# MannLabs/alphadia

Hardware: AMD Instinct MI355X
Metric: precursors scored/sec (higher is better)
Workload: dtype f32/f64; 1 GPU; 1000000-precursor predicted library x 3 candidates vs 2h synthetic Thermo-style DIA run (4800 cycles x 61 spectra); BASELINE configs[2] on one GPU; precursors_total=1000000, candidates_total=3000000, candidates_per_gpu=3000000, cycles=4800, parallelism=single GPU, rccl_ranks_seen=1, priming_steps_before_warmup=4

## Files before the change

### alphadia_amd/csrc/adh_copyout.hip

```cpp

__global__ void adh_slot_count_kernel(const uint16_t *__restrict__ lib_slot, int64_t row0, int64_t n, int top_k,
                                      uint32_t *__restrict__ cnt) {
    const int64_t i = (int64_t)blockIdx.x * blockDim.x + threadIdx.x;
    if (i > n) return;
    uint32_t k = 0;
    if (i < n) {
        const uint16_t *s = lib_slot + (row0 + i) * (int64_t)top_k;
        while (k < (uint32_t)top_k && s[k]) ++k;
    }
    cnt[i] = k;
}

#include "adh_fill_host.h"

struct PadLayout {
    size_t per_row, total;
    PadLayout(int64_t n, int top_k, int64_t n_chunks)
        : per_row(4 + (size_t)top_k * 22), total(base(n, n_chunks + 1, 4 + (size_t)top_k * 22) + 64) {}
    size_t base(int64_t a, int64_t ci) const { return base(a, ci, per_row); }
    static size_t base(int64_t a, int64_t ci, size_t per_row_) {
        return ((size_t)a * per_row_ + ((size_t)(a / kAnchorRows) + (size_t)ci) * 8 + (size_t)ci * 1024 + 255) & ~(size_t)255;
    }
};

// ... 39 lines not shown
        const uint16_t *s = lib_slot + r0;
        for (; v.s < (uint32_t)top_k && s[v.s]; ++v.s) {
            v.i += intensity[r0 + v.s] != 0u;
            v.c += correlation[r0 + v.s] != 0u;
            v.big += s[v.s] >= big_from;
        }
    }
    cnt[i] = v;
}

__global__ void adh_pad_pack_sparse_kernel(DevOut t, int64_t row0, int64_t n, int top_k, const SlotCnt *__restrict__ scan,
                                           unsigned char *__restrict__ block, uint32_t *__restrict__ totals) {
    const int64_t id = (int64_t)blockIdx.x * blockDim.x + threadIdx.x;
    const SlotCnt tot = scan[n];
    const bool sparse = tot.big == 0;
    const SparseBlock L((uint64_t)row0, (uint64_t)n, tot.s, tot.i, tot.c, sparse);
    uint32_t *const off = reinterpret_cast<uint32_t *>(block + L.off);
    if (id == 0) {
        const uint32_t head[4] = {sparse ? kWireSparse : kWireDense, tot.s, tot.i, tot.c};
        for (int q = 0; q < 4; ++q) reinterpret_cast<uint32_t *>(block)[q] = head[q], totals[q] = head[q];
        off[n] = tot.s;
    }
    const bool in_table = id < n * top_k;
    const int64_t i = in_table ? id / top_k : 0;
    const int j = in_table ? (int)(id - i * top_k) : 0;
    SlotCnt a{0, 0, 0, 0};
    uint32_t k = 0;
    if (in_table) {
        a = scan[i];
        k = scan[i + 1].s - a.s;
        if (j == 0) {
            off[i] = a.s;
            if (sparse && (row0 + i) % kAnchorRows == 0) {
                uint32_t *anchor = reinterpret_cast<uint32_t *>(block + L.anchor) +
                                   2 * ((row0 + i) / kAnchorRows - (int64_t)SparseBlock::anchor_row0((uint64_t)row0));
                anchor[0] = a.i, anchor[1] = a.c;
            }
        }
    }
    const bool filled = in_table && (uint32_t)j < k;
    const int64_t src = (row0 + i) * (int64_t)top_k + j;
    const uint32_t *const intensity = reinterpret_cast<const uint32_t *>(t.fragment_intensity);
    const uint32_t *const correlation = reinterpret_cast<const uint32_t *>(t.fragment_correlation);
    const uint32_t vi = filled ? intensity[src] : 0u, vc = filled ? correlation[src] : 0u;
    const uint64_t nz_i = __ballot(vi != 0u), nz_c = __ballot(vc != 0u);
    if (!filled) return;
    const size_t dst = (size_t)a.s + (size_t)j;
    uint16_t word = t.fragment_lib_slot[src];
    size_t di = dst, dc = dst;
    if (sparse) {
        uint32_t pi = a.i, pc = a.c;
        const int lane = (int)(threadIdx.x & (ADH_WAVE - 1));
        if (j <= lane) {
            const uint64_t before = ((1ull << j) - 1ull) << (lane - j);
            pi += (uint32_t)__popcll(nz_i & before), pc += (uint32_t)__popcll(nz_c & before);
        } else {
            for (int q = 0; q < j; ++q) pi += intensity[src - j + q] != 0u, pc += correlation[src - j + q] != 0u;
        }
        di = pi, dc = pc;
        word |= (vi ? kHasIntensity : 0u) | (vc ? kHasCorrelation : 0u);
    }
    reinterpret_cast<uint16_t *>(block + L.slot)[dst] = word;
    reinterpret_cast<float *>(block + L.f[0])[dst] = t.fragment_mz_observed[src];
    reinterpret_cast<float *>(block + L.f[1])[dst] = t.fragment_height[src];
    reinterpret_cast<float *>(block + L.f[3])[dst] = t.fragment_mass_error[src];
    if (!sparse || vi) reinterpret_cast<uint32_t *>(block + L.f[2])[di] = vi;
    if (!sparse || vc) reinterpret_cast<uint32_t *>(block + L.f[4])[dc] = vc;
}

__global__ void adh_cop_count_kernel(const uint8_t *__restrict__ valid, const uint16_t *__restrict__ lib_slot, int64_t row0,
                                     int64_t n, int top_k, uint64_t *__restrict__ cnt) {
    const int64_t i = (int64_t)blockIdx.x * blockDim.x + threadIdx.x;
    if (i > n) return;
    uint64_t v = 0;
    if (i < n && valid[row0 + i]) {
        const uint16_t *s = lib_slot + (row0 + i) * (int64_t)top_k;
        uint32_t k = 0;
        while (k < (uint32_t)top_k && s[k]) ++k;
        v = (1ull << 32) | k;
    }
    cnt[i] = v;
}

struct CopBlock {
    size_t row, cnt, feat, s_slot, s_f[5], total;
    __host__ __device__ CopBlock(uint64_t R, uint64_t S) {
        size_t o = 0;
        row = o, o += (R * 4 + 15) & ~(size_t)15;
        cnt = o, o += (R + 15) & ~(size_t)15;
        feat = o, o += (R * 4 * ADH_NUM_FEATURES + 15) & ~(size_t)15;
        s_slot = o, o += (S * 2 + 15) & ~(size_t)15;
        for (int j = 0; j < 5; ++j) s_f[j] = o, o += (S * 4 + 15) & ~(size_t)15;
        total = o;
    }
};
struct CopLayout {
    size_t per_row, total;
    CopLayout(int64_t n, int top_k, int64_t n_chunks)
        : per_row(5 + 4 * ADH_NUM_FEATURES + (size_t)top_k * 22), total((size_t)n * per_row + (size_t)(n_chunks + 1) * 1024) {}
    size_t base(int64_t a, int64_t ci) const { return ((size_t)a * per_row + (size_t)ci * 1024 + 255) & ~(size_t)255; }
};

__global__ void adh_cop_pack_kernel(DevOut t, DevCands c, const LibRec *__restrict__ lib, int64_t row0, int64_t n, int top_k,
                                    const uint64_t *__restrict__ off, unsigned char *__restrict__ block,
                                    uint64_t *__restrict__ totals) {
    const int64_t stride = (int64_t)gridDim.x * blockDim.x;
    const int64_t tid = (int64_t)blockIdx.x * blockDim.x + threadIdx.x;
    const uint64_t tot = off[n];
    const uint64_t R = tot >> 32, S = tot & 0xFFFFFFFFull;
    if (tid == 0) totals[0] = tot;
    const CopBlock L(R, S);
    uint32_t *const o_row = reinterpret_cast<uint32_t *>(block + L.row);
    uint8_t *const o_cnt = block + L.cnt;
    float *const o_feat = reinterpret_cast<float *>(block + L.feat);
    for (int64_t i = tid; i < n; i += stride) {
        const uint64_t o = off[i], o1 = off[i + 1];
        if ((o1 >> 32) == (o >> 32)) continue;
        const int64_t j = (int64_t)(o >> 32), r = row0 + i;
        o_row[j] = (uint32_t)r;
        o_cnt[j] = (uint8_t)((uint32_t)o1 - (uint32_t)o);
        const float *f = t.features + r * ADH_NUM_FEATURES;
#pragma unroll
        for (int k = 0; k < ADH_NUM_FEATURES; ++k) o_feat[(size_t)k * R + (size_t)j] = f[k];
    }
    uint16_t *const s_slot = reinterpret_cast<uint16_t *>(block + L.s_slot);
    const int64_t n_slots = n * (int64_t)top_k;
    for (int64_t id = tid; id < n_slots; id += stride) {
        const int64_t i = id / top_k;
        const int s = (int)(id - i * top_k);
        const uint64_t o = off[i], o1 = off[i + 1];
        const uint32_t a = (uint32_t)o, k = (uint32_t)o1 - a;
        if ((uint32_t)s >= k) continue;
        const int64_t r = row0 + i, src = r * (int64_t)top_k + s;
        const size_t dst = (size_t)a + (size_t)s;
        s_slot[dst] = t.fragment_lib_slot[src];
        reinterpret_cast<float *>(block + L.s_f[0])[dst] = t.fragment_mz_observed[src];
        reinterpret_cast<float *>(block + L.s_f[1])[dst] = t.fragment_height[src];
        reinterpret_cast<float *>(block + L.s_f[2])[dst] = t.fragment_intensity[src];
        reinterpret_cast<float *>(block + L.s_f[3])[dst] = t.fragment_mass_error[src];
        reinterpret_cast<float *>(block + L.s_f[4])[dst] = t.fragment_correlation[src];
    }
}

namespace {
void cop_copy_stripe(const unsigned char *block, int64_t cnt_r, int64_t cnt_s, int64_t base_r, int64_t base_s,
                     adh_compact_output_t *out, int w, int T, const adh_candidates_t *c, const LibRec *lib) {
    const CopBlock L((uint64_t)cnt_r, (uint64_t)cnt_s);
    const int64_t lo = cnt_r * w / T, hi = cnt_r * (w + 1) / T;
    if (hi <= lo) return;
    const uint32_t *rows = reinterpret_cast<const uint32_t *>(block + L.row);
    const uint8_t *cnt = block + L.cnt;
    int64_t s_lo = 0;
    for (int64_t j = 0; j < lo; ++j) s_lo += cnt[j];
    memcpy(out->row + base_r + lo, rows + lo, (size_t)(hi - lo) * 4);
    const float *fb = reinterpret_cast<const float *>(block + L.feat);
    for (int k = 0; k < ADH_NUM_FEATURES; ++k)
        memcpy(out->features + (size_t)k * (size_t)out->rows_capacity + (size_t)(base_r + lo),
               fb + (size_t)k * (size_t)cnt_r + (size_t)lo, (size_t)(hi - lo) * 4);
    const uint16_t *slot = reinterpret_cast<const uint16_t *>(block + L.s_slot);
    int64_t d = base_s + s_lo, at = s_lo;
    for (int64_t j = lo; j < hi; ++j) {
        const uint32_t r = rows[j];
        const uint32_t p = c->precursor_idx[r];
        const uint8_t rk = c->rank ? c->rank[r] : (uint8_t)0;
        out->precursor_idx[base_r + j] = p;
        out->rank[base_r + j] = rk;
        const LibRec *base = lib + c->frag_start_idx[r];
        const int k = (int)cnt[j];
        for (int q = 0; q < k; ++q, ++d, ++at) {
            const LibRec &l = base[slot[at] - 1];
            out->fragment_row[d] = r;
            out->fragment_precursor_idx[d] = p;
            out->fragment_rank[d] = rk;
            out->fragment_mz_library[d] = l.mz_library;
            out->fragment_mz[d] = l.mz;
            out->fragment_position[d] = l.position;
            out->fragment_number[d] = l.number;
            out->fragment_type[d] = l.type;
            out->fragment_charge[d] = l.charge;
            out->fragment_loss_type[d] = l.loss_type;
        }
    }
    const size_t m = (size_t)(at - s_lo);
    if (m) {
        float *const fcol[5] = {out->fragment_mz_observed, out->fragment_height, out->fragment_intensity, out->fragment_mass_error,
                                out->fragment_correlation};
        for (int j = 0; j < 5; ++j) memcpy(fcol[j] + base_s + s_lo, block + L.s_f[j] + (size_t)s_lo * 4, m * 4);
    }
}

void rebuild_host_rows(const adh_handle *h, const adh_candidates_t *c, adh_output_t *out, const uint16_t *slots,
                       int64_t a, int64_t b) {
    const int top_k = out->top_k;
    const LibRec *lib = h->h_lib.data();
    for (int64_t i = a; i < b; ++i) {
        const bool skip = c->flags && (c->flags[i] & ADH_FLAG_SKIP);
        const uint32_t p = skip ? 0u : c->precursor_idx[i];
        const uint8_t r = skip ? (uint8_t)0 : c->rank[i];
        out->precursor_idx[i] = p;
        out->rank[i] = r;
        const LibRec *base = lib + c->frag_start_idx[i];
        for (int j = 0; j < top_k; ++j) {
            const size_t o = (size_t)i * (size_t)top_k + (size_t)j;
            const uint16_t s = slots[o];
            if (s) {
                const LibRec &l = base[s - 1];
                out->fragment_precursor_idx[o] = p;
                out->fragment_rank[o] = r;
                out->fragment_mz_library[o] = l.mz_library;
                out->fragment_mz[o] = l.mz;
                out->fragment_position[o] = l.position;
                out->fragment_number[o] = l.number;
                out->fragment_type[o] = l.type;
                out->fragment_charge[o] = l.charge;
                out->fragment_loss_type[o] = l.loss_type;
            } else {
                out->fragment_precursor_idx[o] = 0;
                out->fragment_rank[o] = 0;
                out->fragment_mz_library[o] = 0.0f;
                out->fragment_mz[o] = 0.0f;
                out->fragment_position[o] = 0;
                out->fragment_number[o] = 0;
                out->fragment_type[o] = 0;
                out->fragment_charge[o] = 0;
                out->fragment_loss_type[o] = 0;
            }
        }
    }
}

int host_thread_share() {
    int t = 16;
    if (const char *env = getenv("ADH_HOST_THREADS")) t = atoi(env);
    else {
        int ranks = 1;
        if (const char *lw = getenv("LOCAL_WORLD_SIZE")) ranks = std::max(atoi(lw), 1);
        t = std::min<int>(t, std::max<int>(host_cpu_budget() / ranks, 1));
    }
    return std::max(t, 1);
}

int host_threads_for(int64_t n) {
    const int t = (int)std::min<int64_t>(host_thread_share(), n / 16384);
    return std::max(t, 1);
}

bool host_rebuild_pays() {
    int least = 6;
    if (const char *env = getenv("ADH_REBUILD_MIN_THREADS")) least = atoi(env);
    return host_thread_share() >= least;
}

bool compact_copy_out_pays(int64_t n) {
    if (const char *env = getenv("ADH_COMPACT_COPY_OUT")) return atoi(env) != 0;
    int64_t least_rows = 1000000;
    if (const char *env = getenv("ADH_COMPACT_MIN_ROWS")) least_rows = atoll(env);
    return host_thread_share() >= 12 && n >= least_rows;
}

bool sparse_slots_pay(int64_t n) {
    if (const char *env = getenv("ADH_SPARSE_SLOTS")) return atoi(env) != 0;
    int64_t least_rows = 1000000;
    if (const char *env = getenv("ADH_SPARSE_SLOTS_MIN_ROWS")) least_rows = atoll(env);
    return n >= least_rows;
}

struct BlockHandoff {
    std::vector<hipEvent_t> events;
    std::atomic<int64_t> appended{0}, ready{0};
    std::atomic<bool> watching{false}, abort{false};
    hipError_t error = hipSuccess;
    int device = 0;
    std::function<void(int64_t)> landed;
// ... 375 lines not shown
        const int64_t a = cut[(size_t)ci], b = cut[(size_t)ci + 1];
        const double t_in = trace.stripe_begin();
        for (;;) {
            const int64_t t = a / kFillTile + next_tile[(size_t)ci].fetch_add(1, std::memory_order_relaxed);
            const int64_t lo = std::max(a, t * kFillTile), hi = std::min(b, (t + 1) * kFillTile);
            if (lo >= b) break;
            fill_host_rows(h->h_lib.data(), c, out, host_blocks + lay.base(a, ci), b - a, a, lo, hi, sparse);
        }
        trace.stripe_end(ci, w, t_in);
    }
    void start_team() override {
        (void)start_handoff_team(team, T, n_chunks, [this](int64_t ci, int w) { stripe(ci, w); });
    }
    int pack(int64_t ci) override {
        const int64_t a = cut[(size_t)ci], nr = cut[(size_t)ci + 1] - a;
        hipStream_t sk = h->stream;
        unsigned char *blk = dev_blocks + lay.base(a, ci);
        if (sparse) {
            SlotCnt *cnt = static_cast<SlotCnt *>(h->cmp_cnt);
            hipLaunchKernelGGL(adh_slot_count_nz_kernel, dim3((unsigned)((nr + 256) / 256)), dim3(256), 0, sk, dev.fragment_lib_slot,
                               reinterpret_cast<const uint32_t *>(dev.fragment_intensity),
                               reinterpret_cast<const uint32_t *>(dev.fragment_correlation), a, nr, top_k, big_from, cnt);
            size_t scan_bytes = h->cmp_scan_bytes;
            HIP_TRY(hipcub::DeviceScan::ExclusiveScan(h->cmp_scan, scan_bytes, cnt, cnt, SlotCntSum(), SlotCnt{0, 0, 0, 0},
                                                      (int)(nr + 1), sk));
            hipLaunchKernelGGL(adh_pad_pack_sparse_kernel, dim3((unsigned)((nr * top_k + 255) / 256)), dim3(256), 0, sk, dev, a, nr,
                               top_k, cnt, blk, h->cmp_tot_pinned + 4 * ci);
            HIP_TRY(hipGetLastError());
            return record(sk, tot_ready);
        }
        uint32_t *d_off = reinterpret_cast<uint32_t *>(blk);
        hipLaunchKernelGGL(adh_slot_count_kernel, dim3((unsigned)((nr + 256) / 256)), dim3(256), 0, sk, dev.fragment_lib_slot, a,
                           nr, top_k, d_off);
        size_t scan_bytes = h->cmp_scan_bytes;
        HIP_TRY(hipcub::DeviceScan::ExclusiveSum(h->cmp_scan, scan_bytes, d_off, d_off, (int)(nr + 1), sk));
        hipLaunchKernelGGL(adh_pad_pack_kernel, dim3((unsigned)((nr * top_k + 255) / 256)), dim3(256), 0, sk, dev, a, nr, top_k,
                           blk, h->cmp_tot_pinned + ci);
        HIP_TRY(hipGetLastError());
        return record(sk, tot_ready);
    }
    int send(int64_t ci) {
        const int64_t a = cut[(size_t)ci], b = cut[(size_t)ci + 1];
        HIP_TRY(hipEventSynchronize(tot_ready[(size_t)ci]));
        trace.total_seen(ci);
        const size_t base = lay.base(a, ci);
        size_t bytes = 0;
        if (sparse) {
            const uint32_t *tot = h->cmp_tot_pinned + 4 * ci;
            bytes = SparseBlock((uint64_t)a, (uint64_t)(b - a), tot[1], tot[2], tot[3], tot[0] == kWireSparse).total;
            wire_slots += tot[1], wire_nz_i += tot[0] == kWireSparse ? tot[2] : tot[1], wire_nz_c += tot[0] == kWireSparse ? tot[3] : tot[1];
        } else {
            bytes = PadBlock((uint64_t)(b - a), (uint64_t)h->cmp_tot_pinned[ci]).total;
        }
        h->d2h_bytes += bytes;
        trace.block_sent(ci, bytes, PadBlock((uint64_t)(b - a), sparse ? h->cmp_tot_pinned[4 * ci + 1] : h->cmp_tot_pinned[ci]).total);
        return send_block(handoff, host_blocks + base, dev_blocks + base, bytes);
    }
    int copy_out(int64_t ci) override {
        if (ci == 0) {
            HIP_TRY(hipStreamWaitEvent(h->stream_out, h->ev_k[0], 0));
            return copy_tables(0, false);
        }
        int rc = send(ci - 1);
        if (rc == ADH_OK && ci > 1) rc = copy_tables(ci - 1, false);
        return rc;
    }
    int flush() override { return copy_out(n_chunks); }
    int finish() override {
        if (!handoff.wait_for(n_chunks - 1))
            return fail(ADH_ERR_HIP, std::string("scoring pipeline (compacted copy-out): ") + hipGetErrorString(handoff.error));
        for (int64_t ci = 0; ci < n_chunks; ++ci) stripe(ci, T);
        team.join_all();
        if (trace.timing)
            fprintf(stderr, "[adh]   compacted copy-out: host team done %.2f ms after the call began (%d threads)\n", trace.since(), T);
        if (trace.timing && sparse)
            fprintf(stderr, "[adh]   sparse-slot wire: %llu filled slots, %llu intensity words and %llu correlation words sent\n",
                    (unsigned long long)wire_slots, (unsigned long long)wire_nz_i, (unsigned long long)wire_nz_c);
        return ADH_OK;
    }
};

struct OperatorCopyOut : CopyOut {
    adh_compact_output_t *const cop;
    const CopLayout lay;
    const int T;
    int started = 0;
    unsigned char *dev_blocks = nullptr, *stage = nullptr;
    std::vector<int64_t> base_r, base_s, cnt_r, cnt_s;
    bool overflow = false;
    BlockHandoff handoff;
    HandoffTeam team{handoff};
    OperatorCopyOut(const CopyOut &call, adh_compact_output_t *cop_)
        : CopyOut(call), cop(cop_), lay(n, top_k, n_chunks), T(host_threads_for(n)), base_r((size_t)n_chunks + 1, 0),
          base_s((size_t)n_chunks + 1, 0), cnt_r((size_t)n_chunks, 0), cnt_s((size_t)n_chunks, 0),
          handoff(n_chunks, h->device) {}

    void advise_huge_pages() const {
        auto advise = [](void *p, size_t bytes) {
            const uintptr_t lo = ((uintptr_t)p + (2u << 20) - 1) & ~(uintptr_t)((2u << 20) - 1);
            const uintptr_t hi = ((uintptr_t)p + bytes) & ~(uintptr_t)((2u << 20) - 1);
            if (hi > lo) (void)madvise((void *)lo, hi - lo, MADV_HUGEPAGE);
        };
        const size_t rc_ = (size_t)cop->rows_capacity, sc_ = (size_t)cop->slots_capacity;
        advise(cop->features, rc_ * ADH_NUM_FEATURES * 4);
        advise(cop->row, rc_ * 4), advise(cop->precursor_idx, rc_ * 4);
        void *const s4[] = {cop->fragment_row, cop->fragment_precursor_idx, cop->fragment_mz_library, cop->fragment_mz,
                            cop->fragment_mz_observed, cop->fragment_height, cop->fragment_intensity,
                            cop->fragment_mass_error, cop->fragment_correlation};
        for (void *p4 : s4) advise(p4, sc_ * 4);
        void *const s1[] = {cop->fragment_rank, cop->fragment_position, cop->fragment_number, cop->fragment_type,
                            cop->fragment_charge, cop->fragment_loss_type};
        for (void *p1 : s1) advise(p1, sc_);
    }
    int prepare() override {
        if (!compact_output_complete(cop)) return fail(ADH_ERR_INVALID_ARGUMENT, "compact output buffer is NULL");
        advise_huge_pages();
        const size_t cnt_bytes = (size_t)(n + n_chunks) * 8;
        int rc = grow_device(&h->cop_cnt, &h->cop_cnt_bytes, cnt_bytes, cnt_bytes / 8);
        if (rc == ADH_OK) rc = grow_scan_scratch<uint64_t>(&h->cop_scan, &h->cop_scan_bytes, longest_chunk() + 1, h->stream);
        if (rc == ADH_OK) rc = grow_pinned(&h->cop_stage, &h->cop_stage_bytes, lay.total, lay.total / 8);
        if (rc != ADH_OK) return rc;
        if (n_chunks > 4096) return fail(ADH_ERR_UNSUPPORTED, "compact output: more than 4096 chunks");
        if (!h->cop_tot_pinned) HIP_TRY(hipHostMalloc((void **)&h->cop_tot_pinned, 4096 * 8, hipHostMallocDefault));
        rc = grow_device(&h->cop_dev, &h->cop_dev_bytes, lay.total, lay.total / 8 + 4096);
        if (rc != ADH_OK) return rc;
        stage = static_cast<unsigned char *>(h->cop_stage), dev_blocks = static_cast<unsigned char *>(h->cop_dev);
        handoff.landed = [this](int64_t ci) {
            const uint64_t tot = h->cop_tot_pinned[ci];
            base_r[(size_t)ci + 1] = base_r[(size_t)ci] + (int64_t)(tot >> 32);
            base_s[(size_t)ci + 1] = base_s[(size_t)ci] + (int64_t)(tot & 0xFFFFFFFFull);
            if (base_r[(size_t)ci + 1] > cop->rows_capacity || base_s[(size_t)ci + 1] > cop->slots_capacity)
                overflow = true;
            cnt_r[(size_t)ci] = overflow ? 0 : (int64_t)(tot >> 32);
            cnt_s[(size_t)ci] = overflow ? 0 : (int64_t)(tot & 0xFFFFFFFFull);
            if (trace.timing)
                fprintf(stderr, "[adh]   compact chunk %lld: %lld rows, %lld slots on the host %.2f ms after the call began\n",
                        (long long)ci, (long long)(tot >> 32), (long long)(tot & 0xFFFFFFFFull), trace.since());
        };
        return ADH_OK;
    }
    void stripe(int64_t ci, int w) {
        if (cnt_r[(size_t)ci] == 0 && cnt_s[(size_t)ci] == 0) return;
        cop_copy_stripe(stage + lay.base(cut[(size_t)ci], ci), cnt_r[(size_t)ci], cnt_s[(size_t)ci], base_r[(size_t)ci],
                        base_s[(size_t)ci], cop, w, T, c, h->h_lib.data());
    }
    void start_team() override {
        started = start_handoff_team(team, T, n_chunks, [this](int64_t ci, int w) { stripe(ci, w); });
    }
    int pack(int64_t ci) override {
        const int64_t a = cut[(size_t)ci], nr = cut[(size_t)ci + 1] - a;
        hipStream_t sk = h->stream;
        uint64_t *off = static_cast<uint64_t *>(h->cop_cnt) + a + ci;
        hipLaunchKernelGGL(adh_cop_count_kernel, dim3((unsigned)((nr + 256) / 256)), dim3(256), 0, sk, dev.valid,
                           dev.fragment_lib_slot, a, nr, top_k, off);
        size_t scan_bytes = h->cop_scan_bytes;
        HIP_TRY(hipcub::DeviceScan::ExclusiveSum(h->cop_scan, scan_bytes, off, off, (int)(nr + 1), sk));
        hipLaunchKernelGGL(adh_cop_pack_kernel, dim3((unsigned)std::min<int64_t>((nr * top_k + 255) / 256, 8192)), dim3(256), 0,
                           sk, dev, h->cs.d, h->d_lib, a, nr, top_k, off, dev_blocks + lay.base(a, ci), h->cop_tot_pinned + ci);
        HIP_TRY(hipGetLastError());
        return record(sk, tot_ready);
    }
    int send(int64_t ci) {
        HIP_TRY(hipEventSynchronize(tot_ready[(size_t)ci]));
        const uint64_t tot = h->cop_tot_pinned[ci];
        const CopBlock L(tot >> 32, tot & 0xFFFFFFFFull);
        const size_t base = lay.base(cut[(size_t)ci], ci);
        h->d2h_bytes += L.total + 8;
        return send_block(handoff, stage + base, dev_blocks + base, L.total);
    }
    int copy_out(int64_t ci) override {
        return ci > 0 ? send(ci - 1) : ADH_OK;
    }
    int flush() override { return send(n_chunks - 1); }
    int finish() override {
        if (!handoff.wait_for(n_chunks - 1))
            return fail(ADH_ERR_HIP, std::string("scoring pipeline (compact copy-out): ") + hipGetErrorString(handoff.error));
        team.join_all();
        for (int64_t ci = 0; ci < n_chunks; ++ci)
            for (int w = started; w < T; ++w) stripe(ci, w);
        if (trace.timing)
            fprintf(stderr, "[adh]   compact: host team done %.2f ms after the call began (%d threads)\n", trace.since(), T);
        cop->n_rows = base_r[(size_t)n_chunks];
        cop->n_slots = base_s[(size_t)n_chunks];
        if (overflow) {
            (void)hipStreamSynchronize(h->stream);
            (void)hipStreamSynchronize(h->stream_out);
            tables_stand = true;
            return fail(ADH_ERR_INVALID_ARGUMENT, "compact output: rows_capacity / slots_capacity too small (n_rows / n_slots say what is needed)");
        }
        return ADH_OK;
    }
};

}
```

### alphadia_amd/csrc/adh_score_host.hip

```cpp

namespace {

int comm_wait_slot(adh_handle *h, int slot);
int comm_gather_slot(adh_handle *h, int slot);

struct OutFieldDesc {
    const char *name;
    size_t member;
    int per_row;
    int elem;
    bool wire;
    bool optional;
};

const OutFieldDesc kOutFields[] = {
    {"valid", offsetof(adh_output_t, valid), 1, 1, true, false},
    {"features", offsetof(adh_output_t, features), ADH_NUM_FEATURES, 4, true, false},
    {"fragment_mz_observed", offsetof(adh_output_t, fragment_mz_observed), -1, 4, true, false},
    {"fragment_height", offsetof(adh_output_t, fragment_height), -1, 4, true, false},
    {"fragment_intensity", offsetof(adh_output_t, fragment_intensity), -1, 4, true, false},
    {"fragment_mass_error", offsetof(adh_output_t, fragment_mass_error), -1, 4, true, false},
    {"fragment_correlation", offsetof(adh_output_t, fragment_correlation), -1, 4, true, false},
    {"fragment_lib_slot", offsetof(adh_output_t, fragment_lib_slot), -1, 2, true, true},
    {"precursor_idx", offsetof(adh_output_t, precursor_idx), 1, 4, false, false},
// ... 1111 lines not shown
        h->tables_current = rc == ADH_OK;
        return rc;
    }
    std::vector<hipEvent_t> chunk_done, tot_ready;
    PipelineUnwind unwind{h, tab, chunk_done, tot_ready};
    adh_output_t dev = tab.view;
    dev.n = n;
    hipStream_t sk = h->stream, si = h->stream_in;
    HIP_TRY(hipMemsetAsync(tab.base, 0, tab.used, sk));
    tab.partial = false;

    const bool rebuild = !cop && !resident && h->h_lib.size() == (size_t)h->n_lib && !getenv("ADH_DEBUG_COPY_ALL") && host_rebuild_pays();
    const bool compact_wanted = rebuild && top_k <= 65535 && compact_copy_out_pays(n);
    int64_t max_rows = 0;
    if (h->tims_staged) {
        rc = im_chunk_bound(h, c, cfg, &max_rows);
        if (rc != ADH_OK) return rc;
    }
    if (cop || compact_wanted) {
        const int64_t fits_32 = std::max<int64_t>((int64_t)(0xFFFFFFFFull / (uint64_t)top_k) - 1, 1);
        max_rows = max_rows ? std::min(max_rows, fits_32) : fits_32;
    }
    const std::vector<int64_t> cut = chunk_cuts(n, h->tims_staged, max_rows, compact_wanted);
    const int64_t n_chunks = (int64_t)cut.size() - 1;
    const bool compact = compact_wanted && n_chunks <= 4096;
    adh_output_t dev_k = dev;
    if ((rebuild || cop || resident) && !getenv("ADH_DEBUG_WRITE_ALL")) {
        for (int i = 0; i < kNumOutFields; ++i) {
            const OutFieldDesc &f = kOutFields[i];
            if (!f.wire && f.member != offsetof(adh_output_t, stat_matched_peaks)) *out_member(&dev_k, f) = nullptr;
        }
        tab.partial = true;
    }
    const CopyOut call(h, c, dev, cut, chunk_done, tot_ready, trace);
    std::unique_ptr<CopyOut> copy_out;
    if (resident) copy_out.reset(new CopyOut(call));
    else if (cop) copy_out.reset(new OperatorCopyOut(call, cop));
    else if (compact) copy_out.reset(new PackedCopyOut(call, out));
    else copy_out.reset(new PlainCopyOut(call, out, rebuild));
    rc = copy_out->prepare();
    if (rc != ADH_OK) return rc;
    trace.t_1 = trace.now();
    trace.mark_start(si);
    rc = cand_upload_range(h, c, 0, cut[1], si);
    if (rc == ADH_OK) rc = plan_enqueue(h, h->slots[0], cfg, 0, cut[1], si);
    if (rc == ADH_OK && n_chunks > 1) rc = cand_upload_range(h, c, cut[1], cut[2], si);
    if (rc != ADH_OK) return rc;
    copy_out->start_team();
    for (int64_t ci = 0; ci < n_chunks; ++ci) {
        const int64_t a = cut[(size_t)ci], b = cut[(size_t)ci + 1];
        const int ps = (int)(ci & 1);
        if (ci + 1 < n_chunks) {
            const int64_t a2 = b, b2 = cut[(size_t)ci + 2];
            if (ci >= 1) HIP_TRY(hipStreamWaitEvent(si, h->ev_k[ps ^ 1], 0));
            rc = plan_enqueue(h, h->slots[ps ^ 1], cfg, a2, b2 - a2, si);
            if (rc == ADH_OK && ci == 0 && n_chunks > 2) rc = cand_upload_range(h, c, cut[2], cut[3], si);
            if (rc == ADH_OK && ci == 1 && n_chunks > 3) rc = cand_upload_range(h, c, cut[3], n, si);
            if (rc != ADH_OK) return rc;
        }
        Plan p;
        rc = plan_finish(h, h->slots[ps], cfg, a, b - a, p);
        trace.mark(sk);
        if (rc == ADH_OK) rc = launch_scoring(h, p, cfg, &dev_k, sk);
        trace.mark(sk);
        if (rc == ADH_OK) rc = copy_out->pack(ci);
        if (rc != ADH_OK) return rc;
        trace.mark(sk);
        HIP_TRY(hipEventRecord(h->ev_k[ps], sk));
        rc = copy_out->copy_out(ci);
        if (rc != ADH_OK) return rc;
    }
    rc = copy_out->flush();
    if (rc != ADH_OK) return rc;
    trace.t_2 = trace.now();
    rc = comm_gather_slot(h, slot);
    if (rc == ADH_OK) rc = copy_out->finish();
    if (rc != ADH_OK) {
        unwind.ok = h->tables_current = copy_out->tables_stand;
        return rc;
    }
    hipError_t e = hipStreamSynchronize(sk);
    if (e == hipSuccess) e = hipStreamSynchronize(h->stream_out);
    if (e != hipSuccess) return fail(ADH_ERR_HIP, std::string("scoring pipeline: ") + hipGetErrorString(e));
    trace.report(cut, chunk_done, compact);
    unwind.ok = true;
    h->tables_current = true;
    return ADH_OK;
}
}

int adh_score_candidates(adh_handle_t *h, const adh_candidates_t *c, const adh_scoring_config_t *cfg,
                         adh_output_t *out) {
    return score_pipeline(h, c, cfg, out, nullptr);
}

int adh_score_candidates_compact(adh_handle_t *h, const adh_candidates_t *c, const adh_scoring_config_t *cfg,
                                 adh_compact_output_t *cop) {
    if (!h || !c || !cfg || !cop) return fail(ADH_ERR_INVALID_ARGUMENT, "NULL argument");
    if (cop->top_k <= 0 || cop->rows_capacity < 0 || cop->slots_capacity < 0)
        return fail(ADH_ERR_INVALID_ARGUMENT, "compact output: top_k / capacities");
    if (cop->top_k > 255)
        return fail(ADH_ERR_INVALID_ARGUMENT, "compact output: top_k above 255");
    if (h->h_lib.size() != (size_t)h->n_lib)
        return fail(ADH_ERR_NOT_STAGED, "compact output: no host copy of the staged library");
    adh_output_t shape{};
    shape.n = c->n;
    shape.top_k = cop->top_k;
    return score_pipeline(h, c, cfg, &shape, cop);
}

int adh_table_layout(int64_t rows, int32_t top_k, int32_t capacity, adh_table_field_t *fields, int32_t *n_fields,
                     uint64_t *total_bytes, uint64_t *wire_bytes) {
    if (rows < 0 || top_k <= 0 || !n_fields) return fail(ADH_ERR_INVALID_ARGUMENT, "adh_table_layout: bad argument");
    *n_fields = kNumOutFields;
    size_t wire = 0;
    const size_t total = layout_tables(nullptr, rows, top_k, nullptr, &wire);
    if (total_bytes) *total_bytes = total;
    if (wire_bytes) *wire_bytes = wire;
    if (!fields) return ADH_OK;
    if (capacity < kNumOutFields) return fail(ADH_ERR_INVALID_ARGUMENT, "adh_table_layout: field array too short");
    size_t off = 0;
    for (int i = 0; i < kNumOutFields; ++i) {
        const OutFieldDesc &f = kOutFields[i];
        adh_table_field_t &o = fields[i];
        memset(&o, 0, sizeof(o));
        snprintf(o.name, sizeof(o.name), "%s", f.name);
        o.offset = off;
        o.row_elems = (uint32_t)(f.per_row < 0 ? top_k : f.per_row);
        o.elem_bytes = (uint32_t)f.elem;
        o.wire = f.wire ? 1 : 0;
        off += ((size_t)rows * out_row_bytes(f, top_k) + 255) / 256 * 256;
    }
    return ADH_OK;
}

int adh_get_device_tables(adh_handle_t *h, adh_output_t *device_view) {
    if (!h || !device_view) return fail(ADH_ERR_INVALID_ARGUMENT, "NULL argument");
    if (h->last_tables < 0) return fail(ADH_ERR_NOT_STAGED, "no adh_score_candidates call has filled the device tables");
    const int rc = materialise_tables(h);
    if (rc != ADH_OK) return rc;
    *device_view = h->tables[h->last_tables].view;
    device_view->n = h->last_rows;
    return ADH_OK;
}

int adh_debug_get_dense(adh_handle_t *h, int64_t frame_start, int64_t frame_stop, int64_t scan_start, int64_t scan_stop,
                        const float *mz_query, int32_t n_query, float mass_tolerance, float quad_lo, float quad_hi,
                        float *dense, int64_t dense_capacity, int32_t *obs_out, int32_t *n_obs, int32_t *n_scans,
                        int32_t *n_cycles) {
    if (!h || !mz_query || !dense || !obs_out || !n_obs || !n_scans || !n_cycles)
        return fail(ADH_ERR_INVALID_ARGUMENT, "NULL argument");
    if (!h->run_staged && !h->tims_staged) return fail(ADH_ERR_NOT_STAGED, "no run staged");
    if (n_query < 1 || n_query > 4096) return fail(ADH_ERR_INVALID_ARGUMENT, "n_query must be in 1..4096");
    HIP_TRY(hipSetDevice(h->device));
    const bool im = h->tims_staged;
    const int L = im ? h->tims.cycle_len : h->run.cycle_len;
    const int z = im ? h->tims.zeroth : 0;
    const int64_t n_fr = im ? h->tims.n_frames : h->run.n_spectra;
    if (frame_start < z || frame_stop < frame_start || frame_stop > n_fr || (frame_start - z) % L != 0)
        return fail(ADH_ERR_INVALID_ARGUMENT, "frame limits outside the staged run / not on a cycle boundary");
    const int K = n_query;
    const int F = (int)((frame_stop - z) / L - (frame_start - z) / L);
    const int S = im ? (int)(scan_stop - scan_start) : 1;
    if (im && (scan_start < 0 || scan_stop < scan_start || scan_stop > h->tims.scan_max))
        return fail(ADH_ERR_INVALID_ARGUMENT, "scan limits outside the staged run");
    const double *cyc = h->h_cycle.data();
    std::vector<uint16_t> obs;
// ... 234 lines not shown
```

Before: 52.14 million precursors/s.

## Unpack compact output by work-stealing tiles with slot anchors and streaming stores

After: 46.57 million precursors/s. -10.7%, worse.

```diff
diff --git a/alphadia_amd/csrc/adh_copyout.hip b/alphadia_amd/csrc/adh_copyout.hip
--- a/alphadia_amd/csrc/adh_copyout.hip
+++ b/alphadia_amd/csrc/adh_copyout.hip
@@ -145,36 +145,29 @@
     cnt[i] = v;
 }
 
-struct CopBlock {
-    size_t row, cnt, feat, s_slot, s_f[5], total;
-    __host__ __device__ CopBlock(uint64_t R, uint64_t S) {
-        size_t o = 0;
-        row = o, o += (R * 4 + 15) & ~(size_t)15;
-        cnt = o, o += (R + 15) & ~(size_t)15;
-        feat = o, o += (R * 4 * ADH_NUM_FEATURES + 15) & ~(size_t)15;
-        s_slot = o, o += (S * 2 + 15) & ~(size_t)15;
-        for (int j = 0; j < 5; ++j) s_f[j] = o, o += (S * 4 + 15) & ~(size_t)15;
-        total = o;
-    }
-};
+#include "adh_unpack_host.h"
+
 struct CopLayout {
-    size_t per_row, total;
-    CopLayout(int64_t n, int top_k, int64_t n_chunks)
-        : per_row(5 + 4 * ADH_NUM_FEATURES + (size_t)top_k * 22), total((size_t)n * per_row + (size_t)(n_chunks + 1) * 1024) {}
-    size_t base(int64_t a, int64_t ci) const { return ((size_t)a * per_row + (size_t)ci * 1024 + 255) & ~(size_t)255; }
+    size_t per_row, tile, total;
+    CopLayout(int64_t n, int top_k, int64_t n_chunks, int64_t tile_)
+        : per_row(5 + 4 * ADH_NUM_FEATURES + (size_t)top_k * 22), tile((size_t)tile_), total(base(n, n_chunks + 1) + 1024) {}
+    size_t base(int64_t a, int64_t ci) const {
+        return ((size_t)a * per_row + ((size_t)a / tile + (size_t)ci) * 4 + (size_t)ci * 1024 + 255) & ~(size_t)255;
+    }
 };
 
 __global__ void adh_cop_pack_kernel(DevOut t, DevCands c, const LibRec *__restrict__ lib, int64_t row0, int64_t n, int top_k,
-                                    const uint64_t *__restrict__ off, unsigned char *__restrict__ block,
+                                    int64_t tile, const uint64_t *__restrict__ off, unsigned char *__restrict__ block,
                                     uint64_t *__restrict__ totals) {
     const int64_t stride = (int64_t)gridDim.x * blockDim.x;
     const int64_t tid = (int64_t)blockIdx.x * blockDim.x + threadIdx.x;
     const uint64_t tot = off[n];
     const uint64_t R = tot >> 32, S = tot & 0xFFFFFFFFull;
     if (tid == 0) totals[0] = tot;
-    const CopBlock L(R, S);
+    const CopBlock L(R, S, (uint64_t)tile);
     uint32_t *const o_row = reinterpret_cast<uint32_t *>(block + L.row);
     uint8_t *const o_cnt = block + L.cnt;
+    uint32_t *const o_anchor = reinterpret_cast<uint32_t *>(block + L.anchor);
     float *const o_feat = reinterpret_cast<float *>(block + L.feat);
     for (int64_t i = tid; i < n; i += stride) {
         const uint64_t o = off[i], o1 = off[i + 1];
@@ -182,6 +175,7 @@
         const int64_t j = (int64_t)(o >> 32), r = row0 + i;
         o_row[j] = (uint32_t)r;
         o_cnt[j] = (uint8_t)((uint32_t)o1 - (uint32_t)o);
+        if (j % tile == 0) o_anchor[j / tile] = (uint32_t)o;
         const float *f = t.features + r * ADH_NUM_FEATURES;
 #pragma unroll
         for (int k = 0; k < ADH_NUM_FEATURES; ++k) o_feat[(size_t)k * R + (size_t)j] = f[k];
@@ -206,52 +200,6 @@
 }
 
 namespace {
-void cop_copy_stripe(const unsigned char *block, int64_t cnt_r, int64_t cnt_s, int64_t base_r, int64_t base_s,
-                     adh_compact_output_t *out, int w, int T, const adh_candidates_t *c, const LibRec *lib) {
-    const CopBlock L((uint64_t)cnt_r, (uint64_t)cnt_s);
-    const int64_t lo = cnt_r * w / T, hi = cnt_r * (w + 1) / T;
-    if (hi <= lo) return;
-    const uint32_t *rows = reinterpret_cast<const uint32_t *>(block + L.row);
-    const uint8_t *cnt = block + L.cnt;
-    int64_t s_lo = 0;
-    for (int64_t j = 0; j < lo; ++j) s_lo += cnt[j];
-    memcpy(out->row + base_r + lo, rows + lo, (size_t)(hi - lo) * 4);
-    const float *fb = reinterpret_cast<const float *>(block + L.feat);
-    for (int k = 0; k < ADH_NUM_FEATURES; ++k)
-        memcpy(out->features + (size_t)k * (size_t)out->rows_capacity + (size_t)(base_r + lo),
-               fb + (size_t)k * (size_t)cnt_r + (size_t)lo, (size_t)(hi - lo) * 4);
-    const uint16_t *slot = reinterpret_cast<const uint16_t *>(block + L.s_slot);
-    int64_t d = base_s + s_lo, at = s_lo;
-    for (int64_t j = lo; j < hi; ++j) {
-        const uint32_t r = rows[j];
-        const uint32_t p = c->precursor_idx[r];
-        const uint8_t rk = c->rank ? c->rank[r] : (uint8_t)0;
-        out->precursor_idx[base_r + j] = p;
-        out->rank[base_r + j] = rk;
-        const LibRec *base = lib + c->frag_start_idx[r];
-        const int k = (int)cnt[j];
-        for (int q = 0; q < k; ++q, ++d, ++at) {
-            const LibRec &l = base[slot[at] - 1];
-            out->fragment_row[d] = r;
-            out->fragment_precursor_idx[d] = p;
-            out->fragment_rank[d] = rk;
-            out->fragment_mz_library[d] = l.mz_library;
-            out->fragment_mz[d] = l.mz;
-            out->fragment_position[d] = l.position;
-            out->fragment_number[d] = l.number;
-            out->fragment_type[d] = l.type;
-            out->fragment_charge[d] = l.charge;
-            out->fragment_loss_type[d] = l.loss_type;
-        }
-    }
-    const size_t m = (size_t)(at - s_lo);
-    if (m) {
-        float *const fcol[5] = {out->fragment_mz_observed, out->fragment_height, out->fragment_intensity, out->fragment_mass_error,
-                                out->fragment_correlation};
-        for (int j = 0; j < 5; ++j) memcpy(fcol[j] + base_s + s_lo, block + L.s_f[j] + (size_t)s_lo * 4, m * 4);
-    }
-}
-
 void rebuild_host_rows(const adh_handle *h, const adh_candidates_t *c, adh_output_t *out, const uint16_t *slots,
                        int64_t a, int64_t b) {
     const int top_k = out->top_k;
@@ -793,18 +741,19 @@
 
 struct OperatorCopyOut : CopyOut {
     adh_compact_output_t *const cop;
+    const int64_t tile;
     const CopLayout lay;
     const int T;
-    int started = 0;
     unsigned char *dev_blocks = nullptr, *stage = nullptr;
+    std::vector<std::atomic<int64_t>> next_tile;
     std::vector<int64_t> base_r, base_s, cnt_r, cnt_s;
     bool overflow = false;
     BlockHandoff handoff;
     HandoffTeam team{handoff};
     OperatorCopyOut(const CopyOut &call, adh_compact_output_t *cop_)
-        : CopyOut(call), cop(cop_), lay(n, top_k, n_chunks), T(host_threads_for(n)), base_r((size_t)n_chunks + 1, 0),
-          base_s((size_t)n_chunks + 1, 0), cnt_r((size_t)n_chunks, 0), cnt_s((size_t)n_chunks, 0),
-          handoff(n_chunks, h->device) {}
+        : CopyOut(call), cop(cop_), tile(cop_tile_rows()), lay(n, top_k, n_chunks, tile), T(host_threads_for(n)),
+          next_tile((size_t)n_chunks), base_r((size_t)n_chunks + 1, 0), base_s((size_t)n_chunks + 1, 0),
+          cnt_r((size_t)n_chunks, 0), cnt_s((size_t)n_chunks, 0), handoff(n_chunks, h->device) {}
 
     void advise_huge_pages() const {
         auto advise = [](void *p, size_t bytes) {
@@ -836,7 +785,10 @@
         rc = grow_device(&h->cop_dev, &h->cop_dev_bytes, lay.total, lay.total / 8 + 4096);
         if (rc != ADH_OK) return rc;
         stage = static_cast<unsigned char *>(h->cop_stage), dev_blocks = static_cast<unsigned char *>(h->cop_dev);
+        for (std::atomic<int64_t> &next : next_tile) next.store(0, std::memory_order_relaxed);
+        trace.expect_blocks(n_chunks, T);
         handoff.landed = [this](int64_t ci) {
+            trace.team_told(ci);
             const uint64_t tot = h->cop_tot_pinned[ci];
             base_r[(size_t)ci + 1] = base_r[(size_t)ci] + (int64_t)(tot >> 32);
             base_s[(size_t)ci + 1] = base_s[(size_t)ci] + (int64_t)(tot & 0xFFFFFFFFull);
@@ -851,12 +803,18 @@
         return ADH_OK;
     }
     void stripe(int64_t ci, int w) {
-        if (cnt_r[(size_t)ci] == 0 && cnt_s[(size_t)ci] == 0) return;
-        cop_copy_stripe(stage + lay.base(cut[(size_t)ci], ci), cnt_r[(size_t)ci], cnt_s[(size_t)ci], base_r[(size_t)ci],
-                        base_s[(size_t)ci], cop, w, T, c, h->h_lib.data());
+        const int64_t tiles = (int64_t)CopBlock::tiles((uint64_t)cnt_r[(size_t)ci], (uint64_t)tile);
+        const double t_in = trace.stripe_begin();
+        for (;;) {
+            const int64_t t = next_tile[(size_t)ci].fetch_add(1, std::memory_order_relaxed);
+            if (t >= tiles) break;
+            cop_unpack_tile(stage + lay.base(cut[(size_t)ci], ci), cnt_r[(size_t)ci], cnt_s[(size_t)ci], tile, t,
+                            base_r[(size_t)ci], base_s[(size_t)ci], cop, c, h->h_lib.data());
+        }
+        trace.stripe_end(ci, w, t_in);
     }
     void start_team() override {
-        started = start_handoff_team(team, T, n_chunks, [this](int64_t ci, int w) { stripe(ci, w); });
+        (void)start_handoff_team(team, T, n_chunks, [this](int64_t ci, int w) { stripe(ci, w); });
     }
     int pack(int64_t ci) override {
         const int64_t a = cut[(size_t)ci], nr = cut[(size_t)ci + 1] - a;
@@ -867,16 +825,19 @@
         size_t scan_bytes = h->cop_scan_bytes;
         HIP_TRY(hipcub::DeviceScan::ExclusiveSum(h->cop_scan, scan_bytes, off, off, (int)(nr + 1), sk));
         hipLaunchKernelGGL(adh_cop_pack_kernel, dim3((unsigned)std::min<int64_t>((nr * top_k + 255) / 256, 8192)), dim3(256), 0,
-                           sk, dev, h->cs.d, h->d_lib, a, nr, top_k, off, dev_blocks + lay.base(a, ci), h->cop_tot_pinned + ci);
+                           sk, dev, h->cs.d, h->d_lib, a, nr, top_k, tile, off, dev_blocks + lay.base(a, ci),
+                           h->cop_tot_pinned + ci);
         HIP_TRY(hipGetLastError());
         return record(sk, tot_ready);
     }
     int send(int64_t ci) {
         HIP_TRY(hipEventSynchronize(tot_ready[(size_t)ci]));
+        trace.total_seen(ci);
         const uint64_t tot = h->cop_tot_pinned[ci];
-        const CopBlock L(tot >> 32, tot & 0xFFFFFFFFull);
+        const CopBlock L(tot >> 32, tot & 0xFFFFFFFFull, (uint64_t)tile);
         const size_t base = lay.base(cut[(size_t)ci], ci);
         h->d2h_bytes += L.total + 8;
+        trace.block_sent(ci, L.total, L.total);
         return send_block(handoff, stage + base, dev_blocks + base, L.total);
     }
     int copy_out(int64_t ci) override {
@@ -884,11 +845,12 @@
     }
     int flush() override { return send(n_chunks - 1); }
     int finish() override {
-        if (!handoff.wait_for(n_chunks - 1))
-            return fail(ADH_ERR_HIP, std::string("scoring pipeline (compact copy-out): ") + hipGetErrorString(handoff.error));
+        for (int64_t ci = 0; ci < n_chunks; ++ci) {
+            if (!handoff.wait_for(ci))
+                return fail(ADH_ERR_HIP, std::string("scoring pipeline (compact copy-out): ") + hipGetErrorString(handoff.error));
+            stripe(ci, T);
+        }
         team.join_all();
-        for (int64_t ci = 0; ci < n_chunks; ++ci)
-            for (int w = started; w < T; ++w) stripe(ci, w);
         if (trace.timing)
             fprintf(stderr, "[adh]   compact: host team done %.2f ms after the call began (%d threads)\n", trace.since(), T);
         cop->n_rows = base_r[(size_t)n_chunks];
diff --git a/alphadia_amd/csrc/adh_score_host.hip b/alphadia_amd/csrc/adh_score_host.hip
--- a/alphadia_amd/csrc/adh_score_host.hip
+++ b/alphadia_amd/csrc/adh_score_host.hip
@@ -1217,7 +1217,7 @@
     hipError_t e = hipStreamSynchronize(sk);
     if (e == hipSuccess) e = hipStreamSynchronize(h->stream_out);
     if (e != hipSuccess) return fail(ADH_ERR_HIP, std::string("scoring pipeline: ") + hipGetErrorString(e));
-    trace.report(cut, chunk_done, compact);
+    trace.report(cut, chunk_done, compact || cop != nullptr);
     unwind.ok = true;
     h->tables_current = true;
     return ADH_OK;
diff --git a/alphadia_amd/csrc/adh_unpack_host.h b/alphadia_amd/csrc/adh_unpack_host.h
--- /dev/null
+++ b/alphadia_amd/csrc/adh_unpack_host.h
@@ -0,0 +1,126 @@
+#pragma once
+#include <emmintrin.h>
+#include <stdint.h>
+#include <stdlib.h>
+#include <string.h>
+
+#include <algorithm>
+
+#include "adh_device.h"
+
+namespace {
+
+constexpr int64_t kCopTile = 2048;
+inline int64_t cop_tile_rows() {
+    int64_t tile = kCopTile;
+    if (const char *env = getenv("ADH_COP_TILE")) tile = atoll(env);
+    return std::min<int64_t>(std::max<int64_t>(tile, 16), (int64_t)1 << 24);
+}
+
+struct CopBlock {
+    size_t row, cnt, anchor, feat, s_slot, s_f[5], total;
+    __host__ __device__ static uint64_t tiles(uint64_t R, uint64_t tile) { return (R + tile - 1) / tile; }
+    __host__ __device__ CopBlock(uint64_t R, uint64_t S, uint64_t tile) {
+        size_t o = 0;
+        row = o, o += (R * 4 + 15) & ~(size_t)15;
+        cnt = o, o += (R + 15) & ~(size_t)15;
+        anchor = o, o += (tiles(R, tile) * 4 + 15) & ~(size_t)15;
+        feat = o, o += (R * 4 * ADH_NUM_FEATURES + 15) & ~(size_t)15;
+        s_slot = o, o += (S * 2 + 15) & ~(size_t)15;
+        for (int j = 0; j < 5; ++j) s_f[j] = o, o += (S * 4 + 15) & ~(size_t)15;
+        total = o;
+    }
+};
+
+constexpr size_t kCopPrefetch = 1024;
+inline void cop_stream(void *dst, const void *src, size_t bytes) {
+    unsigned char *d = static_cast<unsigned char *>(dst);
+    const unsigned char *s = static_cast<const unsigned char *>(src);
+    const size_t head = std::min<size_t>((size_t)(0 - reinterpret_cast<uintptr_t>(d)) & 15u, bytes);
+    memcpy(d, s, head);
+    d += head, s += head, bytes -= head;
+    size_t q = 0;
+    for (; q + 64 <= bytes; q += 64) {
+        if (q + kCopPrefetch < bytes) _mm_prefetch(reinterpret_cast<const char *>(s + q + kCopPrefetch), _MM_HINT_NTA);
+        const __m128i v0 = _mm_loadu_si128(reinterpret_cast<const __m128i *>(s + q));
+        const __m128i v1 = _mm_loadu_si128(reinterpret_cast<const __m128i *>(s + q + 16));
+        const __m128i v2 = _mm_loadu_si128(reinterpret_cast<const __m128i *>(s + q + 32));
+        const __m128i v3 = _mm_loadu_si128(reinterpret_cast<const __m128i *>(s + q + 48));
+        _mm_stream_si128(reinterpret_cast<__m128i *>(d + q), v0);
+        _mm_stream_si128(reinterpret_cast<__m128i *>(d + q + 16), v1);
+        _mm_stream_si128(reinterpret_cast<__m128i *>(d + q + 32), v2);
+        _mm_stream_si128(reinterpret_cast<__m128i *>(d + q + 48), v3);
+    }
+    for (; q + 16 <= bytes; q += 16)
+        _mm_stream_si128(reinterpret_cast<__m128i *>(d + q), _mm_loadu_si128(reinterpret_cast<const __m128i *>(s + q)));
+    memcpy(d + q, s + q, bytes - q);
+}
+
+void cop_unpack_tile(const unsigned char *block, int64_t cnt_r, int64_t cnt_s, int64_t tile, int64_t t, int64_t base_r,
+                     int64_t base_s, adh_compact_output_t *out, const adh_candidates_t *c, const LibRec *lib) {
+    const int64_t lo = t * tile, hi = std::min(cnt_r, lo + tile);
+    if (t < 0 || lo >= hi) return;
+    const CopBlock L((uint64_t)cnt_r, (uint64_t)cnt_s, (uint64_t)tile);
+    const uint32_t *rows = reinterpret_cast<const uint32_t *>(block + L.row);
+    const uint8_t *cnt = block + L.cnt;
+    const uint32_t *anchor = reinterpret_cast<const uint32_t *>(block + L.anchor);
+    const int64_t s_lo = anchor[t], s_hi = hi < cnt_r ? (int64_t)anchor[t + 1] : cnt_s;
+    const size_t m = (size_t)(hi - lo);
+    cop_stream(out->row + base_r + lo, rows + lo, m * 4);
+    const float *fb = reinterpret_cast<const float *>(block + L.feat);
+    for (int k = 0; k < ADH_NUM_FEATURES; ++k)
+        cop_stream(out->features + (size_t)k * (size_t)out->rows_capacity + (size_t)(base_r + lo),
+                   fb + (size_t)k * (size_t)cnt_r + (size_t)lo, m * 4);
+    if (s_hi > s_lo) {
+        float *const fcol[5] = {out->fragment_mz_observed, out->fragment_height, out->fragment_intensity, out->fragment_mass_error,
+                                out->fragment_correlation};
+        for (int j = 0; j < 5; ++j)
+            cop_stream(fcol[j] + base_s + s_lo, block + L.s_f[j] + (size_t)s_lo * 4, (size_t)(s_hi - s_lo) * 4);
+    }
+    constexpr int kRun = 1024;
+    alignas(64) uint32_t row_p[kRun];
+    alignas(64) uint8_t row_rank[kRun];
+    alignas(64) uint32_t slot_u[2][kRun];
+    alignas(64) float slot_f[2][kRun];
+    alignas(64) uint8_t slot_b[6][kRun];
+    uint32_t *const ucol[2] = {out->fragment_row, out->fragment_precursor_idx};
+    float *const lcol[2] = {out->fragment_mz_library, out->fragment_mz};
+    uint8_t *const bcol[6] = {out->fragment_rank, out->fragment_position, out->fragment_number, out->fragment_type,
+                              out->fragment_charge, out->fragment_loss_type};
+    const uint16_t *slot = reinterpret_cast<const uint16_t *>(block + L.s_slot);
+    int64_t rd = base_r + lo, sd = base_s + s_lo;
+    int64_t r_len = std::min<int64_t>(hi - lo, kRun - (rd & 63)), s_len = std::min<int64_t>(s_hi - s_lo, kRun - (sd & 63));
+    int64_t re = 0, se = 0, at = s_lo;
+    auto put_rows = [&](int64_t len) {
+        cop_stream(out->precursor_idx + rd, row_p, (size_t)len * 4);
+        cop_stream(out->rank + rd, row_rank, (size_t)len);
+        rd += len;
+    };
+    auto put_slots = [&](int64_t len) {
+        for (int j = 0; j < 2; ++j) cop_stream(ucol[j] + sd, slot_u[j], (size_t)len * 4);
+        for (int j = 0; j < 2; ++j) cop_stream(lcol[j] + sd, slot_f[j], (size_t)len * 4);
+        for (int j = 0; j < 6; ++j) cop_stream(bcol[j] + sd, slot_b[j], (size_t)len);
+        sd += len;
+    };
+    for (int64_t j = lo; j < hi; ++j) {
+        const uint32_t r = rows[j];
+        const uint32_t p = c->precursor_idx[r];
+        const uint8_t rk = c->rank ? c->rank[r] : (uint8_t)0;
+        row_p[re] = p, row_rank[re] = rk;
+        if (++re == r_len) put_rows(r_len), re = 0, r_len = std::min<int64_t>(hi - (j + 1), kRun);
+        const LibRec *base = lib + c->frag_start_idx[r];
+        const int64_t end = std::min<int64_t>(at + (int64_t)cnt[j], s_hi);
+        for (; at < end; ++at) {
+            const LibRec &l = base[slot[at] - 1];
+            slot_u[0][se] = r, slot_u[1][se] = p;
+            slot_f[0][se] = l.mz_library, slot_f[1][se] = l.mz;
+            slot_b[0][se] = rk, slot_b[1][se] = l.position, slot_b[2][se] = l.number, slot_b[3][se] = l.type;
+            slot_b[4][se] = l.charge, slot_b[5][se] = l.loss_type;
+            if (++se == s_len) put_slots(s_len), se = 0, s_len = std::min<int64_t>(s_hi - (at + 1), kRun);
+        }
+    }
+    if (se) put_slots(se);
+    _mm_sfence();
+}
+
+}
```
